# ldyken53/gaussian-splatting-wgpu

Hardware: AMD Instinct MI355X
Metric: frames/sec (higher is better)
Workload: dtype f32; 1 GPU; bicycle-like synthetic 6.1M gaussians @1920x1080; gaussians=6100000, width=1920, height=1080, tile_size=16, parallelism=single GPU, visible=2430918, processed=15909895, block_evaluated=6068168, sort_passes=1, depth_ordered_emission=True, tight_binning=True, blend_mode=fused, camera=64-step orbit, moved every frame

## Files before the change

### gaussian-splatting-wgpu_amd/csrc/k_rows.hip

```cpp
#include "gs_device.h"
#include "gs_tight.h"

typedef uint32_t gs_item3 __attribute__((ext_vector_type(3), aligned(4)));

#ifndef RA_ITEMS
#define RA_ITEMS 8
#endif
#ifndef RA_WAVES
#define RA_WAVES 8
#endif
#define RA_THREADS (RA_WAVES * 64)
#define RA_TILE (RA_THREADS * RA_ITEMS)
#define RA_AGG (1u << 30)
#define RA_PREFIX (2u << 30)
#define RA_FLAGS (3u << 30)
#define RA_VALUE (~RA_FLAGS)

#ifndef RB_CH
#define RB_CH 512u
#endif
#define RB_IT (RB_CH / 256u)
#ifndef RB_SB
#define RB_SB 2048u
#endif
#define RB_PER (RB_SB / 256u)
#define RB_WSL (RB_SB / 4u)

struct RowSortShared {
    uint32_t hist[RA_WAVES][256];
    uint32_t gbase[256];
    uint32_t tot[256];
    uint32_t dbase[256];
    uint32_t wsum[RA_WAVES];
    uint32_t tile, nvalid;
    union {
        uint32_t it[RA_TILE * 3];
        struct {
            uint32_t goff[RA_TILE + 8], gptr[RA_TILE + 8];
            unsigned short mark[RA_TILE];
        } g;
    } u;
};

__global__ __launch_bounds__(RA_THREADS) void gs_rows_sort_kernel(const uint32_t* __restrict__ arena, const uint4* __restrict__ grec,
                                                                  const uint32_t* __restrict__ chunk_table, uint32_t* __restrict__ rows_out,
                                                                  GsControl* ctl, uint32_t* __restrict__ status, uint32_t row_cap, uint32_t ndig) {
    __shared__ RowSortShared sh;
    const uint32_t hole = ndig < 128u ? 127u : 255u;
    const int nbits = ndig < 128u ? 7 : 8;
    const uint32_t tid = threadIdx.x, lane = tid & 63, w = tid >> 6;
    const unsigned long long lt_mask = (1ull << lane) - 1ull;
    uint32_t n = ctl->num_slots;
    if (n > row_cap) n = row_cap;
    const uint32_t ntiles = (n + RA_TILE - 1) / RA_TILE;
    const uint32_t nvis = ctl->num_visible;
    {
        const uint32_t c = tid < 256u ? gs_rowhist(ctl, tid) : 0u;
        const uint32_t incl = wave_incl_scan(c, lane);
        if (lane == 63) sh.wsum[w] = incl;
        __syncthreads();
        uint32_t b = 0;
        for (uint32_t k = 0; k < w; ++k) b += sh.wsum[k];
        if (tid < 256u) sh.dbase[tid] = b + incl - c;
        __syncthreads();
    }
    for (;;) {
        if (tid == 0) sh.tile = atomicAdd(&ctl->rows_ticket, 1u);
        __syncthreads();
        const uint32_t tile = sh.tile;
        if (tile >= ntiles) break;
        const uint32_t s0 = tile * RA_TILE, s_end = (s0 + RA_TILE < n) ? s0 + RA_TILE : n;
        const uint32_t g0 = chunk_table[s0 >> 10];
        const uint32_t g1 = (s_end < n) ? chunk_table[s_end >> 10] : nvis - 1u;
        uint32_t K = (g1 >= g0) ? g1 - g0 + 1u : 1u;
        if (K > RA_TILE + 8u) K = RA_TILE + 8u;
        for (uint32_t k = tid; k < RA_TILE / 2u; k += RA_THREADS) reinterpret_cast<uint32_t*>(sh.u.g.mark)[k] = 0u;
        __syncthreads();
        for (uint32_t k = tid; k < K; k += RA_THREADS) {
            const uint4 rec = (g0 + k < nvis) ? grec[g0 + k] : make_uint4(0u, 0u, 0xFFFFFFFFu, 0u);
            sh.u.g.goff[k] = rec.z;
            sh.u.g.gptr[k] = rec.w;
            if (rec.z >= s0 && rec.z < s_end) sh.u.g.mark[rec.z - s0] = (unsigned short)(k + 1u);
        }
        __syncthreads();
        uint32_t carry;
        {
            constexpr uint32_t RA_STR = (RA_TILE + 8u + 63u) / 64u;
            static_assert(RA_STR * 64u >= RA_TILE + 8u && RA_STR <= 128u, "the two-level owner search covers the tile's gaussians");
            const uint32_t x0 = s0 + w * (64 * RA_ITEMS);
            const uint32_t m1 = lane * RA_STR;
            const uint32_t c1 = (uint32_t)__popcll(__ballot(m1 < K && sh.u.g.goff[m1 < K ? m1 : 0u] <= x0));
            const uint32_t b1 = (c1 ? c1 - 1u : 0u) * RA_STR;
            uint32_t c2 = 0;
#pragma unroll
            for (uint32_t t2 = 0; t2 < (RA_STR + 63u) / 64u; ++t2) {
                const uint32_t o2 = t2 * 64u + lane, m2 = b1 + o2;
                c2 += (uint32_t)__popcll(__ballot(o2 < RA_STR && m2 < K && sh.u.g.goff[m2 < K ? m2 : 0u] <= x0));
            }
            const uint32_t e = b1 + (c2 ? c2 - 1u : 0u);
            carry = e + 1u;
        }
        uint32_t ix[RA_ITEMS], iy[RA_ITEMS], iz[RA_ITEMS];
        uint32_t rank2[RA_ITEMS / 2];
#pragma unroll
        for (int j = 0; j < RA_ITEMS; ++j) {
            const uint32_t sp = w * (64 * RA_ITEMS) + j * 64 + lane, slot = s0 + sp;
            uint32_t m = wave_incl_max((uint32_t)sh.u.g.mark[sp]);
            m = m > carry ? m : carry;
            carry = (uint32_t)__builtin_amdgcn_readlane((int)m, 63);
            ix[j] = GS_ROW_HOLE; iy[j] = 0u; iz[j] = 0u;
            if (slot < n) {
                const uint32_t k = m - 1u;
                const uint32_t src = sh.u.g.gptr[k] + (slot - sh.u.g.goff[k]);
                if (src < row_cap) {
                    const gs_item3 v = *reinterpret_cast<const gs_item3*>(arena + (uint64_t)src * 3u);
                    ix[j] = v.x; iy[j] = v.y; iz[j] = v.z;
                }
            }
        }
        for (uint32_t k = lane; k < 256; k += 64) sh.hist[w][k] = 0;
        if (tid < 256u) sh.tot[tid] = 0u;
        __syncthreads();
#pragma unroll
        for (int j = 0; j < RA_ITEMS; ++j) atomicAdd(&sh.tot[ix[j] == GS_ROW_HOLE ? hole : (iy[j] & 0xFFu)], 1u);
        __syncthreads();
        if (tid < ndig) st_agent(status + (uint64_t)tile * 256 + tid, (tile == 0 ? RA_PREFIX : RA_AGG) | sh.tot[tid]);
#pragma unroll
        for (int j = 0; j < RA_ITEMS; ++j) {
            const uint32_t d = ix[j] == GS_ROW_HOLE ? hole : (iy[j] & 0xFFu);
            uint32_t plo = 0xFFFFFFFFu, phi = 0xFFFFFFFFu;
#pragma unroll
            for (int b = 0; b < 8; ++b) {
                if (b < nbits) {
                    const uint32_t bit = (d >> b) & 1u;
                    const unsigned long long bal = __ballot(bit != 0u);
                    const uint32_t inv = bit - 1u;
                    plo &= (uint32_t)bal ^ inv;
                    phi &= (uint32_t)(bal >> 32) ^ inv;
                }
            }
            const uint32_t below = __popc(plo & (uint32_t)lt_mask) + __popc(phi & (uint32_t)(lt_mask >> 32));
            const uint32_t cnt = __popc(plo) + __popc(phi);
            const uint32_t pre = sh.hist[w][d];
            __builtin_amdgcn_fence(__ATOMIC_RELEASE, "wavefront");
            if (below == 0) sh.hist[w][d] = pre + cnt;
            __builtin_amdgcn_fence(__ATOMIC_ACQUIRE, "wavefront");
            const uint32_t r = pre + below;
            if (j & 1) rank2[j >> 1] |= r << 16;
            else rank2[j >> 1] = r;
        }
        __syncthreads();
        uint32_t cw[RA_WAVES], total = 0, excl = 0, incl = 0;
        if (tid < 256u) {
#pragma unroll
            for (int k = 0; k < RA_WAVES; ++k) { cw[k] = sh.hist[k][tid]; total += cw[k]; }
            incl = wave_incl_scan(total, lane);
            if (lane == 63) sh.wsum[w] = incl;
            if (tile > 0 && tid < ndig) {
                constexpr int LB = 8;
                bool found = false;
                for (int t = (int)tile - 1; t >= 0 && !found; t -= LB) {
                    uint32_t sv[LB];
#pragma unroll
                    for (int k = 0; k < LB; ++k) sv[k] = (t - k >= 0) ? ld_agent(status + (uint64_t)(t - k) * 256 + tid) : RA_PREFIX;
#pragma unroll
                    for (int k = 0; k < LB; ++k) {
                        if (found) break;
                        uint32_t v = sv[k], spins = 0;
                        while ((v & RA_FLAGS) == 0 && ++spins < GS_SPIN_LIMIT) {
                            __builtin_amdgcn_s_sleep(1);
                            v = ld_agent(status + (uint64_t)(t - k) * 256 + tid);
                        }
                        if ((v & RA_FLAGS) == 0) { ctl->fault = 1u; found = true; break; }
                        excl += v & RA_VALUE;
                        if ((v & RA_FLAGS) == RA_PREFIX) found = true;
                    }
                }
                st_agent(status + (uint64_t)tile * 256 + tid, RA_PREFIX | ((excl + total) & RA_VALUE));
            }
        }
        __syncthreads();
        if (tid < 256u) {
            uint32_t wv = 0;
            for (uint32_t k = 0; k < w; ++k) wv += sh.wsum[k];
            uint32_t run = wv + incl - total;
            if (tid == hole) sh.nvalid = run;
            sh.gbase[tid] = sh.dbase[tid] + excl - run;
#pragma unroll
            for (int k = 0; k < RA_WAVES; ++k) { sh.hist[k][tid] = run; run += cw[k]; }
        }
        __syncthreads();
#pragma unroll
        for (int j = 0; j < RA_ITEMS; ++j) {
            const uint32_t d = ix[j] == GS_ROW_HOLE ? hole : (iy[j] & 0xFFu);
            const uint32_t r = (j & 1) ? (rank2[j >> 1] >> 16) : (rank2[j >> 1] & 0xFFFFu);
            const uint32_t pos = sh.hist[w][d] + r;
            sh.u.it[pos * 3 + 0] = ix[j];
            sh.u.it[pos * 3 + 1] = iy[j];
            sh.u.it[pos * 3 + 2] = iz[j];
        }
        __syncthreads();
        const uint32_t nvalid = sh.nvalid;
#pragma unroll
        for (int j = 0; j < RA_ITEMS; ++j) {
            const uint32_t pos = j * RA_THREADS + tid;
            if (pos < nvalid) {
                gs_item3 v;
                v.x = sh.u.it[pos * 3 + 0]; v.y = sh.u.it[pos * 3 + 1]; v.z = sh.u.it[pos * 3 + 2];
                const uint32_t g = sh.gbase[v.y & 0xFFu] + pos;
                if (g < row_cap) *reinterpret_cast<gs_item3*>(rows_out + (uint64_t)g * 3u) = v;
            }
        }
        __syncthreads();
    }
}

struct RowTables {
    uint32_t ibase[257];
    uint32_t cbase[257];
    uint32_t w4[8];
};
__device__ __forceinline__ void row_tables(RowTables& T, const GsControl* ctl, uint32_t row_cap, uint32_t tid) {
    const uint32_t lane = tid & 63, w = tid >> 6;
    const bool on = tid < 256u;
    const uint32_t c = on ? gs_rowhist(ctl, tid) : 0u;
    const unsigned long long ic = wave_incl_scan64(c, lane);
    if (on && lane == 63) { T.w4[w] = (uint32_t)(ic > 0xFFFFFFFFull ? 0xFFFFFFFFull : ic); }
    __syncthreads();
    uint32_t i0 = 0, cc = 0;
    if (on) {
        unsigned long long b = ic - c;
        for (uint32_t k = 0; k < w; ++k) b += T.w4[k];
        const unsigned long long e = b + c;
        i0 = b > row_cap ? row_cap : (uint32_t)b;
        const uint32_t i1 = e > row_cap ? row_cap : (uint32_t)e;
        cc = i1 - i0;
        T.ibase[tid] = i0;
        if (tid == 255u) T.ibase[256] = i1;
    }
    const uint32_t ch = (cc + RB_CH - 1u) / RB_CH;
    const uint32_t ih = wave_incl_scan(ch, lane);
    if (on && lane == 63) T.w4[4 + w] = ih;
    __syncthreads();
    if (on) {
        uint32_t bh = 0;
        for (uint32_t k = 0; k < w; ++k) bh += T.w4[4 + k];
        T.cbase[tid] = bh + ih - ch;
        if (tid == 255u) T.cbase[256] = bh + ih;
    }
    __syncthreads();
}
__device__ __forceinline__ uint32_t row_of_chunk(const RowTables& T, uint32_t c) {
    const uint32_t lane = threadIdx.x & 63u;
    uint32_t v[4];
#pragma unroll
    for (int k = 0; k < 4; ++k) v[k] = T.cbase[lane + 64u * k];
    uint32_t r = 0;
#pragma unroll
    for (int k = 0; k < 4; ++k) r += (uint32_t)__popcll(__ballot(v[k] <= c && (lane + 64u * k) != 0u));
    return r;
}

__global__ __launch_bounds__(256) void gs_rows_count_kernel(const uint32_t* __restrict__ rows, const GsControl* ctl, uint32_t* __restrict__ M3,
                                                            uint32_t chunk_cap, uint32_t row_cap) {
    __shared__ RowTables T;
    __shared__ int s_diff[257];
    __shared__ uint32_t s_w[4];
    const uint32_t tid = threadIdx.x, lane = tid & 63, w = tid >> 6;
    row_tables(T, ctl, row_cap, tid);
    uint32_t nch = T.cbase[256];
    if (nch > chunk_cap) nch = chunk_cap;
    for (uint32_t c = blockIdx.x; c < nch; c += gridDim.x) {
        const uint32_t r = row_of_chunk(T, c);
        const uint32_t i0 = T.ibase[r] + (c - T.cbase[r]) * RB_CH;
        const uint32_t i1 = (i0 + RB_CH < T.ibase[r + 1]) ? i0 + RB_CH : T.ibase[r + 1];
        s_diff[tid] = 0;
        if (tid == 0) s_diff[256] = 0;
        __syncthreads();
#pragma unroll
        for (int k = 0; k < (int)(RB_CH / 256u); ++k) {
            const uint32_t i = i0 + k * 256u + tid;
            if (i < i1) {
                const uint32_t w1 = rows[(uint64_t)i * 3u + 1u];
                const uint32_t tlo = (w1 >> 8) & 0xFFu, len = ((w1 >> 16) & 0xFFu) + 1u;
                atomicAdd(&s_diff[tlo], 1);
                atomicAdd(&s_diff[tlo + len > 256u ? 256u : tlo + len], -1);
            }
        }
        __syncthreads();
        const uint32_t v = (uint32_t)s_diff[tid];
        const uint32_t incl = wave_incl_scan(v, lane);
        if (lane == 63) s_w[w] = incl;
        __syncthreads();
        uint32_t b = 0;
        for (uint32_t k = 0; k < w; ++k) b += s_w[k];
        M3[(uint64_t)c * 256u + tid] = b + incl;
        __syncthreads();
    }
}

__global__ __launch_bounds__(1024) void gs_rows_scan_kernel(const GsControl* ctl, uint32_t* __restrict__ M3, uint32_t* __restrict__ tileoff,
                                                            uint32_t* __restrict__ rowtot, uint32_t chunk_cap, uint32_t row_cap) {
    __shared__ RowTables T;
    __shared__ unsigned long long s_part[4][256];
    __shared__ unsigned long long s_ex[256];
    __shared__ unsigned long long s_w[4];
    const uint32_t tid = threadIdx.x, c = tid & 255u, p = tid >> 8, r = blockIdx.x;
    row_tables(T, ctl, row_cap, tid);
    uint32_t c0 = T.cbase[r], c1 = T.cbase[r + 1];
    if (c0 > chunk_cap) c0 = chunk_cap;
    if (c1 > chunk_cap) c1 = chunk_cap;
    const uint32_t nch = c1 - c0, per = (nch + 3u) / 4u;
    const uint32_t j0 = c0 + (p * per < nch ? p * per : nch), j1 = c0 + ((p + 1u) * per < nch ? (p + 1u) * per : nch);
    unsigned long long sum = 0;
    for (uint32_t j = j0; j < j1; j += 8u) {
        uint32_t v[8];
#pragma unroll
        for (int k = 0; k < 8; ++k) v[k] = (j + k < j1) ? M3[(uint64_t)(j + k) * 256u + c] : 0u;
#pragma unroll
        for (int k = 0; k < 8; ++k) sum += v[k];
    }
    s_part[p][c] = sum;
    __syncthreads();
    unsigned long long run = 0, tot = 0;
#pragma unroll
    for (int k = 0; k < 4; ++k) { const unsigned long long t = s_part[k][c]; if (k < (int)p) run += t; tot += t; }
    for (uint32_t j = j0; j < j1; j += 8u) {
        uint32_t v[8];
#pragma unroll
        for (int k = 0; k < 8; ++k) v[k] = (j + k < j1) ? M3[(uint64_t)(j + k) * 256u + c] : 0u;
#pragma unroll
        for (int k = 0; k < 8; ++k) {
            if (j + k < j1) M3[(uint64_t)(j + k) * 256u + c] = run > 0xFFFFFFFFull ? 0xFFFFFFFFu : (uint32_t)run;
            run += v[k];
        }
    }
    if (p == 0) {
        const uint32_t lane = tid & 63, w = tid >> 6;
        unsigned long long incl = tot;
#pragma unroll
        for (int d = 1; d < 64; d <<= 1) {
            const uint32_t lo = __shfl_up((uint32_t)incl, d, 64), hi = __shfl_up((uint32_t)(incl >> 32), d, 64);
            if ((int)lane >= d) incl += ((unsigned long long)hi << 32) | lo;
        }
        if (lane == 63) s_w[w] = incl;
        s_ex[c] = incl - tot;
    }
    __syncthreads();
    if (p == 0) {
        const uint32_t w = tid >> 6;
        unsigned long long b = 0, all = 0;
#pragma unroll
        for (int k = 0; k < 4; ++k) { if (k < (int)w) b += s_w[k]; all += s_w[k]; }
        const unsigned long long ex = b + s_ex[c];
        tileoff[r * 256u + c] = ex > 0xFFFFFFFFull ? 0xFFFFFFFFu : (uint32_t)ex;
        if (c == 0) rowtot[r] = all > 0xFFFFFFFFull ? 0xFFFFFFFFu : (uint32_t)all;
    }
}

struct ExpandShared {
    RowTables T;
    uint32_t rbase[257];
    uint32_t w0[RB_CH], w1[RB_CH], w2[RB_CH];
    uint32_t hist[4][256];
    uint32_t gbase[256];
    uint32_t wsum[8];
    uint32_t nvalid, total;
    unsigned char cols[RB_SB];
    union {
        struct { uint32_t P[RB_CH + 1]; unsigned short mark[RB_SB]; } e;
        uint32_t vals[RB_SB];
    } x;
};

__global__ __launch_bounds__(256) void gs_rows_expand_kernel(const uint32_t* __restrict__ rows, GsControl* ctl, const uint32_t* __restrict__ M3,
                                                             const uint32_t* __restrict__ tileoff, const uint32_t* __restrict__ rowtot, GsFrame f,
                                                             uint32_t* __restrict__ values, uint32_t* __restrict__ ranges, uint32_t chunk_cap,
                                                             uint32_t row_cap, uint32_t* sticky, GsReport* rep) {
    __shared__ ExpandShared S;
    const uint32_t tid = threadIdx.x, lane = tid & 63, w = tid >> 6;
    const unsigned long long lt_mask = (1ull << lane) - 1ull;
    const uint32_t ns = f.tile_size >= 16u ? 2u : 1u;
    const uint32_t hole = f.ntx < 128u ? 127u : 255u;
    const int nbits = f.ntx < 128u ? 7 : 8;
    row_tables(S.T, ctl, row_cap, tid);
    {
        const uint32_t v = tid < f.nty ? rowtot[tid] : 0u;
        unsigned long long incl = v;
#pragma unroll
        for (int d = 1; d < 64; d <<= 1) {
            const uint32_t lo = __shfl_up((uint32_t)incl, d, 64), hi = __shfl_up((uint32_t)(incl >> 32), d, 64);
            if ((int)lane >= d) incl += ((unsigned long long)hi << 32) | lo;
        }
        __shared__ unsigned long long s_r[4];
        if (lane == 63) s_r[w] = incl;
        __syncthreads();
        unsigned long long b = 0;
        for (uint32_t k = 0; k < w; ++k) b += s_r[k];
        const unsigned long long ex = b + incl - v;
        S.rbase[tid] = ex > 0xFFFFFFFFull ? 0xFFFFFFFFu : (uint32_t)ex;
        if (tid == 255u) S.rbase[256] = (b + incl) > 0xFFFFFFFFull ? 0xFFFFFFFFu : (uint32_t)(b + incl);
        __syncthreads();
    }
    if (blockIdx.x == 0 && tid == 0) {
        const uint32_t I = S.rbase[256];
        ctl->num_intersections = I;
        ctl->num_items = S.T.ibase[256];
        if (I > f.capacity) ctl->overflow = 1u;
        gs_frame_report(ctl, I, S.T.ibase[256], f.capacity, sticky, rep);
    }
    for (uint32_t r = blockIdx.x; r < f.nty; r += gridDim.x) {
        if (tid < f.ntx) {
            const uint32_t endoff = (tid + 1u < 256u) ? tileoff[r * 256u + tid + 1u] : rowtot[r];
            const unsigned long long e = (unsigned long long)S.rbase[r] + endoff;
            ranges[r * f.ntx + tid] = e > 0xFFFFFFFFull ? 0xFFFFFFFFu : (uint32_t)e;
        }
    }
    uint32_t nch = S.T.cbase[256];
    if (nch > chunk_cap) nch = chunk_cap;
    gs_item3 nit[RB_IT];
    uint32_t n_r = 0, n_ni = 0, n_tstart = 0, n_done = 0;
    auto prefetch = [&](uint32_t c) {
        n_r = row_of_chunk(S.T, c);
        const uint32_t i0 = S.T.ibase[n_r] + (c - S.T.cbase[n_r]) * RB_CH;
        const uint32_t i1 = (i0 + RB_CH < S.T.ibase[n_r + 1]) ? i0 + RB_CH : S.T.ibase[n_r + 1];
        n_ni = i1 - i0;
#pragma unroll
        for (int k = 0; k < (int)RB_IT; ++k) {
            const uint32_t e = tid * RB_IT + k;
            nit[k] = *reinterpret_cast<const gs_item3*>(rows + (uint64_t)(i0 + (e < n_ni ? e : 0u)) * 3u);
        }
        n_tstart = S.rbase[n_r] + tileoff[n_r * 256u + tid];
        n_done = M3[(uint64_t)c * 256u + tid];
    };
    if (blockIdx.x < nch) prefetch(blockIdx.x);
    for (uint32_t c = blockIdx.x; c < nch; c += gridDim.x) {
        const uint32_t ni = n_ni;
        uint32_t len[RB_IT], lsum = 0;
#pragma unroll
        for (int k = 0; k < (int)RB_IT; ++k) {
            const uint32_t e = tid * RB_IT + k;
            len[k] = 0u;
            if (e < ni) {
                S.w0[e] = nit[k].x; S.w1[e] = nit[k].y; S.w2[e] = nit[k].z;
                len[k] = ((nit[k].y >> 16) & 0xFFu) + 1u;
            }
            lsum += len[k];
        }
        const uint32_t tstart = n_tstart;
        uint32_t done = n_done;
        if (c + gridDim.x < nch) prefetch(c + gridDim.x);
        {
            const uint32_t incl = wave_incl_scan(lsum, lane);
            if (lane == 63) S.wsum[w] = incl;
            __syncthreads();
            uint32_t b = 0, all = 0;
#pragma unroll
            for (int k = 0; k < 4; ++k) { if (k < (int)w) b += S.wsum[k]; all += S.wsum[k]; }
            uint32_t run = b + incl - lsum;
#pragma unroll
            for (int k = 0; k < (int)RB_IT; ++k) { S.x.e.P[tid * RB_IT + k] = run; run += len[k]; }
            if (tid == 0) { S.x.e.P[RB_CH] = all; S.total = all; }
        }
        __syncthreads();
        const uint32_t ninst = S.total;
        for (uint32_t s0 = 0; s0 < ninst; s0 += RB_SB) {
            if (s0) {
                __syncthreads();
                uint32_t l2[RB_IT], ls = 0;
#pragma unroll
                for (int k = 0; k < (int)RB_IT; ++k) { const uint32_t e = tid * RB_IT + k; l2[k] = e < ni ? ((S.w1[e] >> 16) & 0xFFu) + 1u : 0u; ls += l2[k]; }
                const uint32_t incl = wave_incl_scan(ls, lane);
                if (lane == 63) S.wsum[w] = incl;
                __syncthreads();
                uint32_t b = 0;
#pragma unroll
                for (int k = 0; k < 4; ++k) if (k < (int)w) b += S.wsum[k];
                uint32_t run = b + incl - ls;
#pragma unroll
                for (int k = 0; k < (int)RB_IT; ++k) { S.x.e.P[tid * RB_IT + k] = run; run += l2[k]; }
                if (tid == 0) S.x.e.P[RB_CH] = ninst;
            }
            for (uint32_t k = tid; k < RB_SB / 2u; k += 256u) reinterpret_cast<uint32_t*>(S.x.e.mark)[k] = 0u;
            for (uint32_t k = lane; k < 256; k += 64) S.hist[w][k] = 0u;
            __syncthreads();
#pragma unroll
            for (int k = 0; k < (int)RB_IT; ++k) {
                const uint32_t e = tid * RB_IT + k;
                if (e < ni) {
                    const uint32_t p0 = S.x.e.P[e];
                    if (p0 >= s0 && p0 < s0 + RB_SB) S.x.e.mark[p0 - s0] = (unsigned short)(e + 1u);
                }
            }
            __syncthreads();
            uint32_t carry;
            {
                const uint32_t x0 = s0 + w * RB_WSL;
                uint32_t pv[RB_CH / 64u];
#pragma unroll
                for (int k = 0; k < (int)(RB_CH / 64u); ++k) pv[k] = S.x.e.P[lane + 64u * k];
                uint32_t e = 0;
#pragma unroll
                for (int k = 0; k < (int)(RB_CH / 64u); ++k) {
                    const uint32_t m = lane + 64u * k;
                    e += (uint32_t)__popcll(__ballot(m != 0u && m < ni && pv[k] <= x0));
                }
                carry = e + 1u;
            }
            uint32_t val[RB_PER], col4[RB_PER / 4u];
            uint32_t rank2[RB_PER / 2u];
#pragma unroll
            for (int j = 0; j < (int)(RB_PER / 4u); ++j) col4[j] = 0u;
            const uint32_t wfirst = s0 + w * RB_WSL;
            const uint32_t jn = wfirst >= ninst ? 0u : ((ninst - wfirst + 63u) / 64u < RB_PER ? (ninst - wfirst + 63u) / 64u : RB_PER);
#pragma unroll
            for (int j = 0; j < (int)RB_PER; ++j) {
                if ((uint32_t)j >= jn) break;
                const uint32_t sp = w * RB_WSL + j * 64u + lane, x = s0 + sp;
                uint32_t m = wave_incl_max((uint32_t)S.x.e.mark[sp]);
                m = m > carry ? m : carry;
                carry = (uint32_t)__builtin_amdgcn_readlane((int)m, 63);
                uint32_t d = hole;
                val[j] = 0u;
                if (x < ninst) {
                    const uint32_t e = m - 1u;
                    const uint32_t q = x - S.x.e.P[e], i1w = S.w1[e];
                    d = ((i1w >> 8) & 0xFFu) + q;
                    val[j] = (S.w0[e] & GS_ID_MASK) | (tight_item_mask(S.w2[e], q, ns) << GS_ID_BITS);
                }
                col4[j >> 2] |= d << (8 * (j & 3));
            }
#pragma unroll
            for (int j = 0; j < (int)RB_PER; ++j) {
                if ((uint32_t)j >= jn) break;
                const uint32_t d = (col4[j >> 2] >> (8 * (j & 3))) & 0xFFu;
                uint32_t plo = 0xFFFFFFFFu, phi = 0xFFFFFFFFu;
#pragma unroll
                for (int b = 0; b < 8; ++b) {
                    if (b < nbits) {
                        const uint32_t bit = (d >> b) & 1u;
                        const unsigned long long bal = __ballot(bit != 0u);
                        const uint32_t inv = bit - 1u;
                        plo &= (uint32_t)bal ^ inv;
                        phi &= (uint32_t)(bal >> 32) ^ inv;
                    }
                }
                const uint32_t below = __popc(plo & (uint32_t)lt_mask) + __popc(phi & (uint32_t)(lt_mask >> 32));
                const uint32_t cnt = __popc(plo) + __popc(phi);
                const uint32_t pre = S.hist[w][d];
                __builtin_amdgcn_fence(__ATOMIC_RELEASE, "wavefront");
                if (below == 0) S.hist[w][d] = pre + cnt;
                __builtin_amdgcn_fence(__ATOMIC_ACQUIRE, "wavefront");
                const uint32_t rr = pre + below;
                if (j & 1) rank2[j >> 1] |= rr << 16;
                else rank2[j >> 1] = rr;
            }
            __syncthreads();
            {
                uint32_t cw[4], total = 0;
#pragma unroll
                for (int k = 0; k < 4; ++k) { cw[k] = S.hist[k][tid]; total += cw[k]; }
                const uint32_t incl = wave_incl_scan(total, lane);
                if (lane == 63) S.wsum[4 + w] = incl;
                __syncthreads();
                uint32_t b = 0;
#pragma unroll
                for (int k = 0; k < 4; ++k) if (k < (int)w) b += S.wsum[4 + k];
                uint32_t run = b + incl - total;
                if (tid == hole) S.nvalid = run;
                S.gbase[tid] = tstart + done - run;
                done += total;
#pragma unroll
                for (int k = 0; k < 4; ++k) { S.hist[k][tid] = run; run += cw[k]; }
            }
            __syncthreads();
#pragma unroll
            for (int j = 0; j < (int)RB_PER; ++j) {
                if ((uint32_t)j >= jn) break;
                const uint32_t d = (col4[j >> 2] >> (8 * (j & 3))) & 0xFFu;
                const uint32_t rr = (j & 1) ? (rank2[j >> 1] >> 16) : (rank2[j >> 1] & 0xFFFFu);
                const uint32_t pos = S.hist[w][d] + rr;
                S.x.vals[pos] = val[j];
                S.cols[pos] = (unsigned char)d;
            }
            __syncthreads();
            const uint32_t nvalid = S.nvalid;
#pragma unroll
            for (int j = 0; j < (int)RB_PER; ++j) {
                const uint32_t pos = j * 256u + tid;
                if (pos < nvalid) {
                    const uint32_t dst = S.gbase[S.cols[pos]] + pos;
                    if (dst < f.capacity) values[dst] = S.x.vals[pos];
                }
            }
        }
        __syncthreads();
    }
}

__global__ __launch_bounds__(256) void gs_rows_rebuild_keys_kernel(const uint32_t* __restrict__ ranges, uint32_t T, const uint32_t* __restrict__ vals,
                                                                   const uint32_t* __restrict__ counts, uint32_t count, uint32_t n,
                                                                   uint32_t* __restrict__ keys) {
    for (uint32_t i = blockIdx.x * 256u + threadIdx.x; i < count; i += gridDim.x * 256u) {
        uint32_t lo = 0, hi = T;
        while (lo < hi) {
            const uint32_t mid = (lo + hi) >> 1;
            if (ranges[mid] > i) hi = mid; else lo = mid + 1u;
        }
        const uint32_t g = vals[i] & GS_ID_MASK;
        keys[i] = lo * 1000u + (g < n ? counts[g] >> GS_COUNT_BITS : 0u);
    }
}

#ifndef RB_CNT_WG
#define RB_CNT_WG 8u
#endif
#ifndef RB_EXP_WG
#define RB_EXP_WG 6u
#endif
uint32_t gs_rows_sort_tiles(uint64_t row_cap) { return (uint32_t)((row_cap + RA_TILE - 1) / RA_TILE); }
uint32_t gs_rows_chunks(uint64_t row_cap) { return (uint32_t)(row_cap / RB_CH + 256u); }
void gs_launch_rows(const uint32_t* arena, const void* grec, const uint32_t* chunk_table, uint32_t* rows_sorted, GsControl* ctl, uint32_t* sort_status, uint32_t row_cap,
                    uint32_t* M3, uint32_t* tileoff, uint32_t* rowtot, const GsFrame& f, uint32_t* values, uint32_t* ranges, uint32_t cus,
                    uint32_t* sticky, GsReport* rep, hipStream_t st, void (*mark)(void*, int), void* mark_arg) {
    const uint32_t chunk_cap = gs_rows_chunks(row_cap);
    if (!cus) cus = 1;
    hipLaunchKernelGGL(gs_rows_sort_kernel, dim3(cus * 3u), dim3(RA_THREADS), 0, st, arena, (const uint4*)grec, chunk_table, rows_sorted, ctl, sort_status,
                       row_cap, f.nty);
    if (mark) mark(mark_arg, 3);
    hipLaunchKernelGGL(gs_rows_count_kernel, dim3(cus * RB_CNT_WG), dim3(256), 0, st, (const uint32_t*)rows_sorted, (const GsControl*)ctl, M3, chunk_cap, row_cap);
    hipLaunchKernelGGL(gs_rows_scan_kernel, dim3(f.nty), dim3(1024), 0, st, (const GsControl*)ctl, M3, tileoff, rowtot, chunk_cap, row_cap);
    hipLaunchKernelGGL(gs_rows_expand_kernel, dim3(cus * RB_EXP_WG), dim3(256), 0, st, (const uint32_t*)rows_sorted, ctl, (const uint32_t*)M3,
                       (const uint32_t*)tileoff, (const uint32_t*)rowtot, f, values, ranges, chunk_cap, row_cap, sticky, rep);
}
void gs_launch_rows_rebuild_keys(const uint32_t* ranges, uint32_t T, const uint32_t* vals, const uint32_t* counts, uint32_t count, uint32_t n,
                                 uint32_t* keys, hipStream_t st) {
    if (!count) return;
    const uint32_t blocks = (count + 255u) / 256u;
    hipLaunchKernelGGL(gs_rows_rebuild_keys_kernel, dim3(blocks < 4096u ? blocks : 4096u), dim3(256), 0, st, ranges, T, vals, counts, count, n, keys);
}
```

### gaussian-splatting-wgpu_amd/csrc/gs_device.h

```cpp
#pragma once
#include <hip/hip_runtime.h>
#include <stdint.h>

#define GS_WAVE 64

struct GsFrame {
    uint32_t n;
    uint32_t width, height, tile_size;
    uint32_t ntx, nty;
    uint32_t col0, col1;
    uint32_t px0, slab_w;
    uint32_t capacity;
    uint32_t full;
    uint32_t row_cap;
};

#define GS_COUNT_BITS 22
#define GS_COUNT_MASK 0x3FFFFFu

struct GsControl {
    uint32_t scan_ticket[2];
    uint32_t sort_ticket[4];
    uint32_t rows_ticket;
    uint32_t num_slots;
    uint32_t num_items;
    uint32_t fault;
    uint32_t overflow;
    uint32_t num_intersections;
    uint32_t num_visible;
    uint32_t pad0;
    uint32_t row_cursor[16];
    unsigned long long num_processed[64];
    unsigned long long num_evaluated[64];
    uint32_t hist[4][256];
    uint32_t rowhist[8][256];
};
__device__ __forceinline__ uint32_t gs_rowhist(const GsControl* ctl, uint32_t r) {
    uint32_t s = 0;
#pragma unroll
    for (int k = 0; k < 8; ++k) s += ctl->rowhist[k][r];
    return s;
}

struct GsReport {
    uint32_t fault, overflow, num_intersections, num_visible, num_slots, num_items, pad0, pad1;
    uint32_t row_cursor[16];
    uint32_t sticky[4];
};
__device__ __forceinline__ void gs_frame_report(const GsControl* ctl, uint32_t I, uint32_t num_items, uint32_t capacity, uint32_t* sticky,
                                                GsReport* rep) {
    uint32_t need = 0;
    for (int k = 0; k < 16; ++k) need = ctl->row_cursor[k] > need ? ctl->row_cursor[k] : need;
    need = need > 0x07FFFFFFu ? 0x7FFFFFFFu : need * 16u;
    const uint32_t over = (I > capacity || ctl->overflow) ? 1u : 0u;
    uint32_t s0 = 0, s1 = 0, s2 = 0, s3 = 0;
    if (sticky) {
        s0 = atomicAdd(&sticky[0], over) + over;
        s1 = atomicOr(&sticky[1], ctl->fault ? 1u : 0u) | (ctl->fault ? 1u : 0u);
        s2 = atomicMax(&sticky[2], I); s2 = s2 > I ? s2 : I;
        s3 = atomicMax(&sticky[3], need); s3 = s3 > need ? s3 : need;
    }
    if (rep) {
        rep->fault = ctl->fault; rep->overflow = over; rep->num_intersections = I; rep->num_visible = ctl->num_visible;
        rep->num_slots = ctl->num_slots; rep->num_items = num_items;
        for (int k = 0; k < 16; ++k) rep->row_cursor[k] = ctl->row_cursor[k];
        rep->sticky[0] = s0; rep->sticky[1] = s1; rep->sticky[2] = s2; rep->sticky[3] = s3;
    }
}

struct GsTightOut {
    uint32_t* arena; uint32_t* rowptr; GsControl* ctl;
};

struct GsScene {
    const float* px; const float* py; const float* pz;
    const float* smax;
    const float4* geo;
    const float4* sh;
    const uint8_t* state;
};

#define GS_ST_HIDDEN 1u
#define GS_ST_SELECTED 2u
struct GsTint { float t[3]; float k; };

struct GsPlyTable {
    uint32_t stride, nsrc, all_float;
    uint16_t soff[11 + 48];
    uint8_t stype[11 + 48], slot[11 + 48];
};

struct GsUniforms {
    float view[16];
    float proj[16];
    float cam[3];
    float tan_fovx, tan_fovy, focal_x, focal_y, scale_modifier;
};

__device__ __forceinline__ float wg_max(float a, float b) { return (a < b) ? b : a; }
__device__ __forceinline__ float wg_min(float a, float b) { return (b < a) ? b : a; }
__device__ __forceinline__ int wg_maxi(int a, int b) { return (a < b) ? b : a; }
__device__ __forceinline__ int wg_mini(int a, int b) { return (b < a) ? b : a; }

__device__ __forceinline__ int f2i_sat(float x) {
    if (x != x) return 0;
    if (x >= 2147483648.0f) return 2147483647;
    if (x <= -2147483648.0f) return (-2147483647 - 1);
    return (int)x;
}
__device__ __forceinline__ uint32_t f2u_sat(float x) {
    if (x != x) return 0u;
    if (x >= 4294967296.0f) return 0xFFFFFFFFu;
    if (x <= 0.0f) return 0u;
    return (uint32_t)x;
}

__device__ __forceinline__ float gs_exp(float x) {
    if (x != x) return x;
    if (x > 88.72283935546875f) return __builtin_inff();
    if (x < -103.97208404541015625f) return 0.0f;
    const float nf = __builtin_rintf(x * 1.44269502162933349609375f);
    float r = __builtin_fmaf(-nf, 0.693145751953125f, x);
    r = __builtin_fmaf(-nf, 1.42860677465796470642e-06f, r);
    float p = 1.9875691500e-4f;
    p = __builtin_fmaf(p, r, 1.3981999507e-3f);
    p = __builtin_fmaf(p, r, 8.3334519073e-3f);
    p = __builtin_fmaf(p, r, 4.1665795894e-2f);
    p = __builtin_fmaf(p, r, 1.6666665459e-1f);
    p = __builtin_fmaf(p, r, 5.0000001201e-1f);
    const float z = r * r;
    float y = __builtin_fmaf(p, z, r);
    y = y + 1.0f;
    const int n = (int)nf;
    const int a = n >> 1;
    const int b = n - a;
    const float sa = __uint_as_float((uint32_t)(a + 127) << 23);
    const float sb = __uint_as_float((uint32_t)(b + 127) << 23);
    return (y * sa) * sb;
}

__device__ __forceinline__ void slab_cols(uint32_t rx0, uint32_t rx1, const GsFrame& f, uint32_t& xa, uint32_t& wmain,
                                          uint32_t& alias) {
    const uint32_t hi = rx1 < f.ntx ? rx1 : f.ntx;
    xa = rx0 > f.col0 ? rx0 : f.col0;
    const uint32_t xb = hi < f.col1 ? hi : f.col1;
    wmain = xb > xa ? xb - xa : 0u;
    alias = (rx1 == f.ntx + 1u && f.col0 == 0u) ? 1u : 0u;
}

__device__ __forceinline__ uint32_t lane_id() { return __builtin_amdgcn_mbcnt_hi(~0u, __builtin_amdgcn_mbcnt_lo(~0u, 0u)); }

#define GS_DPP(v, ctrl, rm) (uint32_t)__builtin_amdgcn_update_dpp(0, (int)(v), (ctrl), (rm), 0xf, false)
__device__ __forceinline__ uint32_t wave_incl_scan(uint32_t v, uint32_t) {
    v += GS_DPP(v, 0x111, 0xf);
    v += GS_DPP(v, 0x112, 0xf);
    v += GS_DPP(v, 0x114, 0xf);
    v += GS_DPP(v, 0x118, 0xf);
    v += GS_DPP(v, 0x142, 0xa);
    v += GS_DPP(v, 0x143, 0xc);
    return v;
}
__device__ __forceinline__ unsigned long long wave_incl_scan64(unsigned long long v, uint32_t lane) {
#pragma unroll
    for (int d = 1; d < 64; d <<= 1) {
        const uint32_t lo = __shfl_up((uint32_t)v, d, 64), hi = __shfl_up((uint32_t)(v >> 32), d, 64);
        if ((int)lane >= d) v += ((unsigned long long)hi << 32) | lo;
    }
    return v;
}
__device__ __forceinline__ uint32_t wave_incl_max(uint32_t v) {
    uint32_t t;
    t = GS_DPP(v, 0x111, 0xf); v = (t > v) ? t : v;
    t = GS_DPP(v, 0x112, 0xf); v = (t > v) ? t : v;
    t = GS_DPP(v, 0x114, 0xf); v = (t > v) ? t : v;
    t = GS_DPP(v, 0x118, 0xf); v = (t > v) ? t : v;
    t = GS_DPP(v, 0x142, 0xa); v = (t > v) ? t : v;
    t = GS_DPP(v, 0x143, 0xc); v = (t > v) ? t : v;
    return v;
}
__device__ __forceinline__ uint32_t wave_sum(uint32_t v) {
    return (uint32_t)__builtin_amdgcn_readlane((int)wave_incl_scan(v, 0u), 63);
}

__device__ __forceinline__ void st_agent(uint32_t* p, uint32_t v) {
    __hip_atomic_store(p, v, __ATOMIC_RELAXED, __HIP_MEMORY_SCOPE_AGENT);
}
__device__ __forceinline__ uint32_t ld_agent(const uint32_t* p) {
    return __hip_atomic_load(p, __ATOMIC_RELAXED, __HIP_MEMORY_SCOPE_AGENT);
}
__device__ __forceinline__ void st_agent64(unsigned long long* p, unsigned long long v) {
    __hip_atomic_store(p, v, __ATOMIC_RELAXED, __HIP_MEMORY_SCOPE_AGENT);
}
__device__ __forceinline__ unsigned long long ld_agent64(const unsigned long long* p) {
    return __hip_atomic_load(p, __ATOMIC_RELAXED, __HIP_MEMORY_SCOPE_AGENT);
}

#define GS_SPIN_LIMIT (1u << 22)
```

Before: 1365 frames/s.

## Prefetch next row-sort tile records and store sorted rows as planar arrays

The row sort kernel now grabs its next tile ticket early and prefetches that tile's chunk bounds and gaussian records into registers while the current tile scatters. This hides global-load latency between tiles. Sorted rows move from an interleaved 3-word layout to three planar arrays, so the count and expand kernels read coalesced single words. The sort grid size now comes from the occupancy API instead of a fixed 3 blocks per CU, and the expand kernel gets a launch-bounds occupancy hint. These add register pressure, and the kernel relies on the planar layout having room for 3*row_cap words.

```diff
diff --git a/gaussian-splatting-wgpu_amd/csrc/k_rows.hip b/gaussian-splatting-wgpu_amd/csrc/k_rows.hip
--- a/gaussian-splatting-wgpu_amd/csrc/k_rows.hip
+++ b/gaussian-splatting-wgpu_amd/csrc/k_rows.hip
@@ -11,6 +11,9 @@
 #endif
 #define RA_THREADS (RA_WAVES * 64)
 #define RA_TILE (RA_THREADS * RA_ITEMS)
+#ifndef RA_PF
+#define RA_PF 4
+#endif
 #define RA_AGG (1u << 30)
 #define RA_PREFIX (2u << 30)
 #define RA_FLAGS (3u << 30)
@@ -50,10 +53,38 @@
     const int nbits = ndig < 128u ? 7 : 8;
     const uint32_t tid = threadIdx.x, lane = tid & 63, w = tid >> 6;
     const unsigned long long lt_mask = (1ull << lane) - 1ull;
+    uint32_t* const rows_w0 = rows_out;
+    uint32_t* const rows_w1 = rows_out + (size_t)row_cap;
+    uint32_t* const rows_w2 = rows_out + (size_t)row_cap * 2u;
     uint32_t n = ctl->num_slots;
     if (n > row_cap) n = row_cap;
     const uint32_t ntiles = (n + RA_TILE - 1) / RA_TILE;
     const uint32_t nvis = ctl->num_visible;
+    uint32_t g0 = 0, g1 = 0;
+    uint2 nrec[RA_PF ? RA_PF : 1];
+    auto tile_bounds = [&](uint32_t t) {
+        if (t < ntiles) {
+            const uint32_t t0 = t * RA_TILE, t1 = (t0 + RA_TILE < n) ? t0 + RA_TILE : n;
+            g0 = chunk_table[t0 >> 10];
+            g1 = (t1 < n) ? chunk_table[t1 >> 10] : nvis - 1u;
+        }
+    };
+    auto tile_count = [&]() {
+        const uint32_t K = (g1 >= g0) ? g1 - g0 + 1u : 1u;
+        return K > RA_TILE + 8u ? RA_TILE + 8u : K;
+    };
+    auto tile_records = [&](uint32_t t) {
+        if (t < ntiles) {
+            const uint32_t K = tile_count();
+#pragma unroll
+            for (int i = 0; i < RA_PF; ++i) {
+                const uint32_t k = i * RA_THREADS + tid;
+                nrec[i] = make_uint2(0xFFFFFFFFu, 0u);
+                if (k < K && g0 + k < nvis) nrec[i] = reinterpret_cast<const uint2*>(grec + (g0 + k))[1];
+            }
+        }
+    };
+    if (tid == 0) sh.tile = atomicAdd(&ctl->rows_ticket, 1u);
     {
         const uint32_t c = tid < 256u ? gs_rowhist(ctl, tid) : 0u;
         const uint32_t incl = wave_incl_scan(c, lane);
@@ -64,23 +95,32 @@
         if (tid < 256u) sh.dbase[tid] = b + incl - c;
         __syncthreads();
     }
-    for (;;) {
-        if (tid == 0) sh.tile = atomicAdd(&ctl->rows_ticket, 1u);
-        __syncthreads();
-        const uint32_t tile = sh.tile;
-        if (tile >= ntiles) break;
+    uint32_t tile = sh.tile;
+    tile_bounds(tile);
+    tile_records(tile);
+    while (tile < ntiles) {
         const uint32_t s0 = tile * RA_TILE, s_end = (s0 + RA_TILE < n) ? s0 + RA_TILE : n;
-        const uint32_t g0 = chunk_table[s0 >> 10];
-        const uint32_t g1 = (s_end < n) ? chunk_table[s_end >> 10] : nvis - 1u;
-        uint32_t K = (g1 >= g0) ? g1 - g0 + 1u : 1u;
-        if (K > RA_TILE + 8u) K = RA_TILE + 8u;
+        const uint32_t K = tile_count(), cg0 = g0;
         for (uint32_t k = tid; k < RA_TILE / 2u; k += RA_THREADS) reinterpret_cast<uint32_t*>(sh.u.g.mark)[k] = 0u;
-        __syncthreads();
-        for (uint32_t k = tid; k < K; k += RA_THREADS) {
-            const uint4 rec = (g0 + k < nvis) ? grec[g0 + k] : make_uint4(0u, 0u, 0xFFFFFFFFu, 0u);
-            sh.u.g.goff[k] = rec.z;
-            sh.u.g.gptr[k] = rec.w;
-            if (rec.z >= s0 && rec.z < s_end) sh.u.g.mark[rec.z - s0] = (unsigned short)(k + 1u);
+#pragma unroll
+        for (int i = 0; i < RA_PF; ++i) {
+            const uint32_t k = i * RA_THREADS + tid;
+            if (k < K) { sh.u.g.goff[k] = nrec[i].x; sh.u.g.gptr[k] = nrec[i].y; }
+        }
+        for (uint32_t k = RA_PF * RA_THREADS + tid; k < K; k += RA_THREADS) {
+            const uint2 rec = (cg0 + k < nvis) ? reinterpret_cast<const uint2*>(grec + (cg0 + k))[1] : make_uint2(0xFFFFFFFFu, 0u);
+            sh.u.g.goff[k] = rec.x;
+            sh.u.g.gptr[k] = rec.y;
+        }
+        __syncthreads();
+#pragma unroll
+        for (int i = 0; i < RA_PF; ++i) {
+            const uint32_t k = i * RA_THREADS + tid, z = nrec[i].x;
+            if (k < K && z >= s0 && z < s_end) sh.u.g.mark[z - s0] = (unsigned short)(k + 1u);
+        }
+        for (uint32_t k = RA_PF * RA_THREADS + tid; k < K; k += RA_THREADS) {
+            const uint32_t z = sh.u.g.goff[k];
+            if (z >= s0 && z < s_end) sh.u.g.mark[z - s0] = (unsigned short)(k + 1u);
         }
         __syncthreads();
         uint32_t carry;
@@ -179,7 +219,10 @@
                 st_agent(status + (uint64_t)tile * 256 + tid, RA_PREFIX | ((excl + total) & RA_VALUE));
             }
         }
-        __syncthreads();
+        uint32_t ticket = 0;
+        if (tid == 0) ticket = atomicAdd(&ctl->rows_ticket, 1u);
+        __syncthreads();
+        if (tid == 0) sh.tile = ticket;
         if (tid < 256u) {
             uint32_t wv = 0;
             for (uint32_t k = 0; k < w; ++k) wv += sh.wsum[k];
@@ -190,6 +233,8 @@
             for (int k = 0; k < RA_WAVES; ++k) { sh.hist[k][tid] = run; run += cw[k]; }
         }
         __syncthreads();
+        const uint32_t next = sh.tile;
+        tile_bounds(next);
 #pragma unroll
         for (int j = 0; j < RA_ITEMS; ++j) {
             const uint32_t d = ix[j] == GS_ROW_HOLE ? hole : (iy[j] & 0xFFu);
@@ -200,6 +245,7 @@
             sh.u.it[pos * 3 + 2] = iz[j];
         }
         __syncthreads();
+        tile_records(next);
         const uint32_t nvalid = sh.nvalid;
 #pragma unroll
         for (int j = 0; j < RA_ITEMS; ++j) {
@@ -208,10 +254,11 @@
                 gs_item3 v;
                 v.x = sh.u.it[pos * 3 + 0]; v.y = sh.u.it[pos * 3 + 1]; v.z = sh.u.it[pos * 3 + 2];
                 const uint32_t g = sh.gbase[v.y & 0xFFu] + pos;
-                if (g < row_cap) *reinterpret_cast<gs_item3*>(rows_out + (uint64_t)g * 3u) = v;
-            }
-        }
-        __syncthreads();
+                if (g < row_cap) { rows_w0[g] = v.x; rows_w1[g] = v.y; rows_w2[g] = v.z; }
+            }
+        }
+        __syncthreads();
+        tile = next;
     }
 }
 
@@ -267,6 +314,7 @@
     __shared__ int s_diff[257];
     __shared__ uint32_t s_w[4];
     const uint32_t tid = threadIdx.x, lane = tid & 63, w = tid >> 6;
+    const uint32_t* const rows_w1 = rows + (size_t)row_cap;
     row_tables(T, ctl, row_cap, tid);
     uint32_t nch = T.cbase[256];
     if (nch > chunk_cap) nch = chunk_cap;
@@ -281,7 +329,7 @@
         for (int k = 0; k < (int)(RB_CH / 256u); ++k) {
             const uint32_t i = i0 + k * 256u + tid;
             if (i < i1) {
-                const uint32_t w1 = rows[(uint64_t)i * 3u + 1u];
+                const uint32_t w1 = rows_w1[i];
                 const uint32_t tlo = (w1 >> 8) & 0xFFu, len = ((w1 >> 16) & 0xFFu) + 1u;
                 atomicAdd(&s_diff[tlo], 1);
                 atomicAdd(&s_diff[tlo + len > 256u ? 256u : tlo + len], -1);
@@ -373,7 +421,7 @@
     } x;
 };
 
-__global__ __launch_bounds__(256) void gs_rows_expand_kernel(const uint32_t* __restrict__ rows, GsControl* ctl, const uint32_t* __restrict__ M3,
+__global__ __launch_bounds__(256, 6) void gs_rows_expand_kernel(const uint32_t* __restrict__ rows, GsControl* ctl, const uint32_t* __restrict__ M3,
                                                              const uint32_t* __restrict__ tileoff, const uint32_t* __restrict__ rowtot, GsFrame f,
                                                              uint32_t* __restrict__ values, uint32_t* __restrict__ ranges, uint32_t chunk_cap,
                                                              uint32_t row_cap, uint32_t* sticky, GsReport* rep) {
@@ -383,6 +431,8 @@
     const uint32_t ns = f.tile_size >= 16u ? 2u : 1u;
     const uint32_t hole = f.ntx < 128u ? 127u : 255u;
     const int nbits = f.ntx < 128u ? 7 : 8;
+    const uint32_t* const rows_w1 = rows + (size_t)row_cap;
+    const uint32_t* const rows_w2 = rows + (size_t)row_cap * 2u;
     row_tables(S.T, ctl, row_cap, tid);
     {
         const uint32_t v = tid < f.nty ? rowtot[tid] : 0u;
@@ -428,7 +478,8 @@
 #pragma unroll
         for (int k = 0; k < (int)RB_IT; ++k) {
             const uint32_t e = tid * RB_IT + k;
-            nit[k] = *reinterpret_cast<const gs_item3*>(rows + (uint64_t)(i0 + (e < n_ni ? e : 0u)) * 3u);
+            const uint32_t i = i0 + (e < n_ni ? e : 0u);
+            nit[k].x = rows[i]; nit[k].y = rows_w1[i]; nit[k].z = rows_w2[i];
         }
         n_tstart = S.rbase[n_r] + tileoff[n_r * 256u + tid];
         n_done = M3[(uint64_t)c * 256u + tid];
@@ -620,12 +671,20 @@
 #endif
 uint32_t gs_rows_sort_tiles(uint64_t row_cap) { return (uint32_t)((row_cap + RA_TILE - 1) / RA_TILE); }
 uint32_t gs_rows_chunks(uint64_t row_cap) { return (uint32_t)(row_cap / RB_CH + 256u); }
+static uint32_t rows_sort_residency() {
+    static const uint32_t per_cu = [] {
+        int nb = 0;
+        if (hipOccupancyMaxActiveBlocksPerMultiprocessor(&nb, gs_rows_sort_kernel, RA_THREADS, 0) != hipSuccess || nb < 1) { (void)hipGetLastError(); nb = 2; }
+        return (uint32_t)(nb > 4 ? 4 : nb);
+    }();
+    return per_cu;
+}
 void gs_launch_rows(const uint32_t* arena, const void* grec, const uint32_t* chunk_table, uint32_t* rows_sorted, GsControl* ctl, uint32_t* sort_status, uint32_t row_cap,
                     uint32_t* M3, uint32_t* tileoff, uint32_t* rowtot, const GsFrame& f, uint32_t* values, uint32_t* ranges, uint32_t cus,
                     uint32_t* sticky, GsReport* rep, hipStream_t st, void (*mark)(void*, int), void* mark_arg) {
     const uint32_t chunk_cap = gs_rows_chunks(row_cap);
     if (!cus) cus = 1;
-    hipLaunchKernelGGL(gs_rows_sort_kernel, dim3(cus * 3u), dim3(RA_THREADS), 0, st, arena, (const uint4*)grec, chunk_table, rows_sorted, ctl, sort_status,
+    hipLaunchKernelGGL(gs_rows_sort_kernel, dim3(cus * rows_sort_residency()), dim3(RA_THREADS), 0, st, arena, (const uint4*)grec, chunk_table, rows_sorted, ctl, sort_status,
                        row_cap, f.nty);
     if (mark) mark(mark_arg, 3);
     hipLaunchKernelGGL(gs_rows_count_kernel, dim3(cus * RB_CNT_WG), dim3(256), 0, st, (const uint32_t*)rows_sorted, (const GsControl*)ctl, M3, chunk_cap, row_cap);
```

Result: no change. 1367 frames/s (median of 2 runs) (+0.2%).

## Replace ballot-based wave digit ranking with LDS bitmap atomics in row sort/expand

Applied to the files above, without the earlier changes.

Within-wave digit ranking in the row sort and expand kernels used to rely on 7-8 ballot passes per item. It now sets a bit in a per-wave, per-digit 64-bit LDS bitmap with an atomic OR, reads the bitmap back, and popcounts it to get both the rank and the count. Hole items are skipped instead of ranked, and the expand kernel's histogram shrinks to 16-bit entries. The bitmap storage in the expand kernel is dynamic shared memory sized from ntx, and the grid size is recomputed from an LDS budget. This trades ballot ALU work for LDS atomics, which may contend when many lanes share a digit, and the larger LDS footprint may reduce the number of resident workgroups.

```diff
diff --git a/gaussian-splatting-wgpu_amd/csrc/gs_device.h b/gaussian-splatting-wgpu_amd/csrc/gs_device.h
--- a/gaussian-splatting-wgpu_amd/csrc/gs_device.h
+++ b/gaussian-splatting-wgpu_amd/csrc/gs_device.h
@@ -182,6 +182,19 @@
     return (uint32_t)__builtin_amdgcn_readlane((int)wave_incl_scan(v, 0u), 63);
 }
 
+__device__ __forceinline__ void wave_rank_bitmap(unsigned long long* bm_row, uint32_t d, uint32_t lane, unsigned long long lt_mask,
+                                                 uint32_t& below, uint32_t& cnt) {
+    __builtin_amdgcn_fence(__ATOMIC_ACQ_REL, "wavefront");
+    __hip_atomic_fetch_or(reinterpret_cast<uint32_t*>(bm_row + d) + (lane >> 5), 1u << (lane & 31u), __ATOMIC_RELAXED, __HIP_MEMORY_SCOPE_WORKGROUP);
+    __builtin_amdgcn_fence(__ATOMIC_ACQ_REL, "wavefront");
+    const unsigned long long m = __hip_atomic_load(bm_row + d, __ATOMIC_RELAXED, __HIP_MEMORY_SCOPE_WORKGROUP);
+    __builtin_amdgcn_fence(__ATOMIC_ACQ_REL, "wavefront");
+    below = (uint32_t)__popcll(m & lt_mask);
+    cnt = (uint32_t)__popcll(m);
+    if (below == 0) __hip_atomic_store(bm_row + d, 0ull, __ATOMIC_RELAXED, __HIP_MEMORY_SCOPE_WORKGROUP);
+    __builtin_amdgcn_fence(__ATOMIC_ACQ_REL, "wavefront");
+}
+
 __device__ __forceinline__ void st_agent(uint32_t* p, uint32_t v) {
     __hip_atomic_store(p, v, __ATOMIC_RELAXED, __HIP_MEMORY_SCOPE_AGENT);
 }
diff --git a/gaussian-splatting-wgpu_amd/csrc/k_rows.hip b/gaussian-splatting-wgpu_amd/csrc/k_rows.hip
--- a/gaussian-splatting-wgpu_amd/csrc/k_rows.hip
+++ b/gaussian-splatting-wgpu_amd/csrc/k_rows.hip
@@ -39,6 +39,7 @@
             uint32_t goff[RA_TILE + 8], gptr[RA_TILE + 8];
             unsigned short mark[RA_TILE];
         } g;
+        unsigned long long bm[RA_WAVES][256];
     } u;
 };
 
@@ -126,26 +127,21 @@
         __syncthreads();
         if (tid < ndig) st_agent(status + (uint64_t)tile * 256 + tid, (tile == 0 ? RA_PREFIX : RA_AGG) | sh.tot[tid]);
 #pragma unroll
+        for (int k = 0; k < 4; ++k)
+            if (k < (nbits == 7 ? 2 : 4)) sh.u.bm[w][lane + 64u * k] = 0ull;
+#pragma unroll
         for (int j = 0; j < RA_ITEMS; ++j) {
-            const uint32_t d = ix[j] == GS_ROW_HOLE ? hole : (iy[j] & 0xFFu);
-            uint32_t plo = 0xFFFFFFFFu, phi = 0xFFFFFFFFu;
-#pragma unroll
-            for (int b = 0; b < 8; ++b) {
-                if (b < nbits) {
-                    const uint32_t bit = (d >> b) & 1u;
-                    const unsigned long long bal = __ballot(bit != 0u);
-                    const uint32_t inv = bit - 1u;
-                    plo &= (uint32_t)bal ^ inv;
-                    phi &= (uint32_t)(bal >> 32) ^ inv;
-                }
-            }
-            const uint32_t below = __popc(plo & (uint32_t)lt_mask) + __popc(phi & (uint32_t)(lt_mask >> 32));
-            const uint32_t cnt = __popc(plo) + __popc(phi);
-            const uint32_t pre = sh.hist[w][d];
-            __builtin_amdgcn_fence(__ATOMIC_RELEASE, "wavefront");
-            if (below == 0) sh.hist[w][d] = pre + cnt;
-            __builtin_amdgcn_fence(__ATOMIC_ACQUIRE, "wavefront");
-            const uint32_t r = pre + below;
+            uint32_t r = 0u;
+            if (ix[j] != GS_ROW_HOLE) {
+                const uint32_t d = iy[j] & 0xFFu;
+                uint32_t below, cnt;
+                const uint32_t pre = sh.hist[w][d];
+                wave_rank_bitmap(sh.u.bm[w], d, lane, lt_mask, below, cnt);
+                __builtin_amdgcn_fence(__ATOMIC_RELEASE, "wavefront");
+                if (below == 0) sh.hist[w][d] = pre + cnt;
+                __builtin_amdgcn_fence(__ATOMIC_ACQUIRE, "wavefront");
+                r = pre + below;
+            }
             if (j & 1) rank2[j >> 1] |= r << 16;
             else rank2[j >> 1] = r;
         }
@@ -192,7 +188,8 @@
         __syncthreads();
 #pragma unroll
         for (int j = 0; j < RA_ITEMS; ++j) {
-            const uint32_t d = ix[j] == GS_ROW_HOLE ? hole : (iy[j] & 0xFFu);
+            if (ix[j] == GS_ROW_HOLE) continue;
+            const uint32_t d = iy[j] & 0xFFu;
             const uint32_t r = (j & 1) ? (rank2[j >> 1] >> 16) : (rank2[j >> 1] & 0xFFFFu);
             const uint32_t pos = sh.hist[w][d] + r;
             sh.u.it[pos * 3 + 0] = ix[j];
@@ -362,9 +359,9 @@
     RowTables T;
     uint32_t rbase[257];
     uint32_t w0[RB_CH], w1[RB_CH], w2[RB_CH];
-    uint32_t hist[4][256];
+    unsigned short hist[4][256];
     uint32_t gbase[256];
-    uint32_t wsum[8];
+    union { uint32_t wsum[8]; unsigned long long s_r[4]; };
     uint32_t nvalid, total;
     unsigned char cols[RB_SB];
     union {
@@ -373,16 +370,18 @@
     } x;
 };
 
-__global__ __launch_bounds__(256) void gs_rows_expand_kernel(const uint32_t* __restrict__ rows, GsControl* ctl, const uint32_t* __restrict__ M3,
+__global__ __launch_bounds__(256) __attribute__((amdgpu_waves_per_eu(6))) void gs_rows_expand_kernel(const uint32_t* __restrict__ rows, GsControl* ctl, const uint32_t* __restrict__ M3,
                                                              const uint32_t* __restrict__ tileoff, const uint32_t* __restrict__ rowtot, GsFrame f,
                                                              uint32_t* __restrict__ values, uint32_t* __restrict__ ranges, uint32_t chunk_cap,
                                                              uint32_t row_cap, uint32_t* sticky, GsReport* rep) {
     __shared__ ExpandShared S;
+    extern __shared__ unsigned long long s_bm[];
     const uint32_t tid = threadIdx.x, lane = tid & 63, w = tid >> 6;
     const unsigned long long lt_mask = (1ull << lane) - 1ull;
     const uint32_t ns = f.tile_size >= 16u ? 2u : 1u;
-    const uint32_t hole = f.ntx < 128u ? 127u : 255u;
-    const int nbits = f.ntx < 128u ? 7 : 8;
+    const uint32_t hole = 255u;
+    unsigned long long* const bm_row = s_bm + w * f.ntx;
+    for (uint32_t k = tid; k < 4u * f.ntx; k += 256u) s_bm[k] = 0ull;
     row_tables(S.T, ctl, row_cap, tid);
     {
         const uint32_t v = tid < f.nty ? rowtot[tid] : 0u;
@@ -392,11 +391,10 @@
             const uint32_t lo = __shfl_up((uint32_t)incl, d, 64), hi = __shfl_up((uint32_t)(incl >> 32), d, 64);
             if ((int)lane >= d) incl += ((unsigned long long)hi << 32) | lo;
         }
-        __shared__ unsigned long long s_r[4];
-        if (lane == 63) s_r[w] = incl;
+        if (lane == 63) S.s_r[w] = incl;
         __syncthreads();
         unsigned long long b = 0;
-        for (uint32_t k = 0; k < w; ++k) b += s_r[k];
+        for (uint32_t k = 0; k < w; ++k) b += S.s_r[k];
         const unsigned long long ex = b + incl - v;
         S.rbase[tid] = ex > 0xFFFFFFFFull ? 0xFFFFFFFFu : (uint32_t)ex;
         if (tid == 255u) S.rbase[256] = (b + incl) > 0xFFFFFFFFull ? 0xFFFFFFFFu : (uint32_t)(b + incl);
@@ -482,7 +480,7 @@
                 if (tid == 0) S.x.e.P[RB_CH] = ninst;
             }
             for (uint32_t k = tid; k < RB_SB / 2u; k += 256u) reinterpret_cast<uint32_t*>(S.x.e.mark)[k] = 0u;
-            for (uint32_t k = lane; k < 256; k += 64) S.hist[w][k] = 0u;
+            for (uint32_t k = lane; k < 128; k += 64) reinterpret_cast<uint32_t*>(S.hist[w])[k] = 0u;
             __syncthreads();
 #pragma unroll
             for (int k = 0; k < (int)RB_IT; ++k) {
@@ -534,24 +532,16 @@
             for (int j = 0; j < (int)RB_PER; ++j) {
                 if ((uint32_t)j >= jn) break;
                 const uint32_t d = (col4[j >> 2] >> (8 * (j & 3))) & 0xFFu;
-                uint32_t plo = 0xFFFFFFFFu, phi = 0xFFFFFFFFu;
-#pragma unroll
-                for (int b = 0; b < 8; ++b) {
-                    if (b < nbits) {
-                        const uint32_t bit = (d >> b) & 1u;
-                        const unsigned long long bal = __ballot(bit != 0u);
-                        const uint32_t inv = bit - 1u;
-                        plo &= (uint32_t)bal ^ inv;
-                        phi &= (uint32_t)(bal >> 32) ^ inv;
-                    }
+                uint32_t rr = 0u;
+                if (d < f.ntx) {
+                    uint32_t below, cnt;
+                    const uint32_t pre = S.hist[w][d];
+                    wave_rank_bitmap(bm_row, d, lane, lt_mask, below, cnt);
+                    __builtin_amdgcn_fence(__ATOMIC_RELEASE, "wavefront");
+                    if (below == 0) S.hist[w][d] = (unsigned short)(pre + cnt);
+                    __builtin_amdgcn_fence(__ATOMIC_ACQUIRE, "wavefront");
+                    rr = pre + below;
                 }
-                const uint32_t below = __popc(plo & (uint32_t)lt_mask) + __popc(phi & (uint32_t)(lt_mask >> 32));
-                const uint32_t cnt = __popc(plo) + __popc(phi);
-                const uint32_t pre = S.hist[w][d];
-                __builtin_amdgcn_fence(__ATOMIC_RELEASE, "wavefront");
-                if (below == 0) S.hist[w][d] = pre + cnt;
-                __builtin_amdgcn_fence(__ATOMIC_ACQUIRE, "wavefront");
-                const uint32_t rr = pre + below;
                 if (j & 1) rank2[j >> 1] |= rr << 16;
                 else rank2[j >> 1] = rr;
             }
@@ -571,13 +561,14 @@
                 S.gbase[tid] = tstart + done - run;
                 done += total;
 #pragma unroll
-                for (int k = 0; k < 4; ++k) { S.hist[k][tid] = run; run += cw[k]; }
+                for (int k = 0; k < 4; ++k) { S.hist[k][tid] = (unsigned short)run; run += cw[k]; }
             }
             __syncthreads();
 #pragma unroll
             for (int j = 0; j < (int)RB_PER; ++j) {
                 if ((uint32_t)j >= jn) break;
                 const uint32_t d = (col4[j >> 2] >> (8 * (j & 3))) & 0xFFu;
+                if (d >= f.ntx) continue;
                 const uint32_t rr = (j & 1) ? (rank2[j >> 1] >> 16) : (rank2[j >> 1] & 0xFFFFu);
                 const uint32_t pos = S.hist[w][d] + rr;
                 S.x.vals[pos] = val[j];
@@ -630,7 +621,10 @@
     if (mark) mark(mark_arg, 3);
     hipLaunchKernelGGL(gs_rows_count_kernel, dim3(cus * RB_CNT_WG), dim3(256), 0, st, (const uint32_t*)rows_sorted, (const GsControl*)ctl, M3, chunk_cap, row_cap);
     hipLaunchKernelGGL(gs_rows_scan_kernel, dim3(f.nty), dim3(1024), 0, st, (const GsControl*)ctl, M3, tileoff, rowtot, chunk_cap, row_cap);
-    hipLaunchKernelGGL(gs_rows_expand_kernel, dim3(cus * RB_EXP_WG), dim3(256), 0, st, (const uint32_t*)rows_sorted, ctl, (const uint32_t*)M3,
+    const uint32_t bm_bytes = 4u * f.ntx * 8u;
+    const uint32_t lds_wg = (uint32_t)((sizeof(ExpandShared) + bm_bytes + 1279u) / 1280u) * 1280u;
+    const uint32_t exp_wg = std::min<uint32_t>(RB_EXP_WG, 163840u / lds_wg);
+    hipLaunchKernelGGL(gs_rows_expand_kernel, dim3(cus * exp_wg), dim3(256), bm_bytes, st, (const uint32_t*)rows_sorted, ctl, (const uint32_t*)M3,
                        (const uint32_t*)tileoff, (const uint32_t*)rowtot, f, values, ranges, chunk_cap, row_cap, sticky, rep);
 }
 void gs_launch_rows_rebuild_keys(const uint32_t* ranges, uint32_t T, const uint32_t* vals, const uint32_t* counts, uint32_t count, uint32_t n,
```

After: 1320 frames/s before, 1327 frames/s after (median of 6 runs). No clear change (+0.5%).
